# ameli/gaussian-process-param-estimation

Measured on NVIDIA B200. Metric: loglik+grad evals/s (Matern nu=2.5 dense n=20k, FP64), higher is better.
Workload: dtype f64

## Files before the change

gaussian-process-param-estimation_b200/csrc/gp_loglik.cu:

```cuda
#include "../../include/gpgp.h"
#include "gp_common.cuh"
#include "gp_internal.h"
#include "gp_matern.cuh"

namespace gp {

constexpr int MAXP = 16;
constexpr int LMAXD = 8;

__global__ void __launch_bounds__(256)
gram_partial_kernel(const double* __restrict__ A, const double* __restrict__ B, int nrows, int p, int64_t ld,
                    double* partial) {
    __shared__ double sa[64 * MAXP], sb[64 * MAXP];
    const int tid = threadIdx.x;
    const int a = tid / p, b = tid - a * p;
    double acc = 0.0;
    int rows_per_cta = (nrows + gridDim.x - 1) / gridDim.x;
    int r0 = blockIdx.x * rows_per_cta, r1 = min(nrows, r0 + rows_per_cta);
    for (int base = r0; base < r1; base += 64) {
        int cnt = min(64, r1 - base);
        __syncthreads();
        for (int idx = tid; idx < cnt * p; idx += 256) {
            int r = idx / p, c = idx - r * p;
            sa[idx] = A[(int64_t)(base + r) * ld + c];
            sb[idx] = B[(int64_t)(base + r) * ld + c];
        }
        __syncthreads();
        if (tid < p * p)
            for (int r = 0; r < cnt; ++r) acc += sa[r * p + a] * sb[r * p + b];
    }
    if (tid < p * p) partial[(int64_t)blockIdx.x * p * p + tid] = acc;
}

__global__ void sum_partials_kernel(const double* partial, int nparts, int width, double* out) {
    int t = blockIdx.x * blockDim.x + threadIdx.x;
    if (t >= width) return;
    double s = 0.0;
    for (int i = 0; i < nparts; ++i) s += partial[(int64_t)i * width + t];
    out[t] = s;
}

template <int MODE, bool WITH_DK>
__global__ void __launch_bounds__(256)
trace_tiles_kernel(const double* __restrict__ Ainv, int n, int npad, const double* __restrict__ pts, int d,
                   MaternParams mp, double* partial) {
    __shared__ double pr[LMAXD][128], pc[LMAXD][128];
    __shared__ double red[32];
    int b = blockIdx.x;
    int tm = (int)((sqrt(8.0 * b + 1.0) - 1.0) * 0.5);
    while ((tm + 1) * (tm + 2) / 2 <= b) ++tm;
    while (tm * (tm + 1) / 2 > b) --tm;
    int tn = b - tm * (tm + 1) / 2;
    const int m0 = tm * 128, n0 = tn * 128, tid = threadIdx.x;
    if (WITH_DK) {
        for (int idx = tid; idx < 128 * d; idx += 256) {
            int r = idx / d, k = idx - r * d;
            pr[k][r] = (m0 + r < n) ? pts[(int64_t)(m0 + r) * d + k] : 0.0;
            pc[k][r] = (n0 + r < n) ? pts[(int64_t)(n0 + r) * d + k] : 0.0;
        }
        __syncthreads();
    }
    double t1 = 0.0, t2 = 0.0, t3 = 0.0;
    const int tx = tid & 63, ty = tid >> 6;
    for (int r = ty; r < 128; r += 4) {
        int gi = m0 + r;
        if (gi >= n) break;
        double2 v = *reinterpret_cast<const double2*>(Ainv + (int64_t)gi * npad + n0 + 2 * tx);
        double vals[2] = {v.x, v.y};
#pragma unroll
        for (int e = 0; e < 2; ++e) {
            int gj = n0 + 2 * tx + e;
            if (gj > gi || gj >= n) continue;
            double a = vals[e];
            if (gj == gi) {
                t1 += a;
                t2 += a * a;
            } else {
                t2 += 2.0 * a * a;
                if (WITH_DK) {
                    double s = 0.0, ud = 0.0;
#pragma unroll
                    for (int k = 0; k < LMAXD; ++k)
                        if (k < d) {
                            double t = (pr[k][r] - pc[k][2 * tx + e]) * mp.inv_scale[k];
                            s += t * t;
                            if (k == mp.ddim) ud = t * t;
                        }
                    double val, dval;
                    matern_value_drho<MODE>(sqrt(s), mp, &val, &dval);
                    if (mp.ddim >= 0) dval = (s > 0.0) ? dval * (ud / s) * mp.inv_scale[mp.ddim] : 0.0;
                    t3 += 2.0 * a * dval;
                }
            }
        }
    }
    t1 = block_sum(t1, red);
    t2 = block_sum(t2, red);
    t3 = block_sum(t3, red);
    if (tid == 0) {
        partial[(int64_t)b * 3 + 0] = t1;
        partial[(int64_t)b * 3 + 1] = t2;
        partial[(int64_t)b * 3 + 2] = t3;
    }
}

__global__ void __launch_bounds__(256)
frob_lower_kernel(const double* __restrict__ W, int n, int npad, double* partial) {
    __shared__ double red[32];
    int tm = blockIdx.y, tn = blockIdx.x;
    double s = 0.0;
    if (tn <= tm) {
        int m0 = tm * 128, n0 = tn * 128;
        for (int idx = threadIdx.x; idx < 128 * 64; idx += 256) {
            int r = idx >> 6, c = (idx & 63) * 2;
            int gi = m0 + r;
            if (gi >= n) break;
            double2 v = *reinterpret_cast<const double2*>(W + (int64_t)gi * npad + n0 + c);
            if (n0 + c <= gi) s += v.x * v.x;
            if (n0 + c + 1 <= gi) s += v.y * v.y;
        }
    }
    s = block_sum(s, red);
    if (threadIdx.x == 0) partial[blockIdx.y * gridDim.x + blockIdx.x] = s;
}

constexpr int SSP = MAXP + 1;
constexpr int DKR = 16;
template <int MODE, int PP>
__global__ void __launch_bounds__(256)
dk_apply_kernel(const double* __restrict__ pts, int n, int d, MaternParams mp, const double* __restrict__ S, int p,
                int64_t lds, double* __restrict__ V) {
    constexpr int SP = PP + 1;
    __shared__ double pcs[LMAXD][128];
    __shared__ double ss[128 * SP];
    const int tid = threadIdx.x, lane = tid & 31, warp = tid >> 5;
    const int g0 = blockIdx.x * DKR + warp * 2;
    double pi[2][LMAXD];
#pragma unroll
    for (int r = 0; r < 2; ++r)
#pragma unroll
        for (int k = 0; k < LMAXD; ++k) pi[r][k] = (k < d && g0 + r < n) ? pts[(int64_t)(g0 + r) * d + k] : 0.0;
    double acc[2][PP];
#pragma unroll
    for (int r = 0; r < 2; ++r)
#pragma unroll
        for (int c = 0; c < PP; ++c) acc[r][c] = 0.0;
    for (int j0 = 0; j0 < n; j0 += 128) {
        __syncthreads();
        for (int idx = tid; idx < 128 * d; idx += 256) {
            int r = idx / d, k = idx - r * d;
            pcs[k][r] = (j0 + r < n) ? pts[(int64_t)(j0 + r) * d + k] : 0.0;
        }
        for (int idx = tid; idx < 128 * p; idx += 256) {
            int r = idx / p, c = idx - r * p;
            ss[r * SP + c] = (j0 + r < n) ? S[(int64_t)(j0 + r) * lds + c] : 0.0;
        }
        __syncthreads();
#pragma unroll
        for (int t = 0; t < 4; ++t) {
            const int jj = t * 32 + lane;
            const int gj = j0 + jj;
#pragma unroll
            for (int r = 0; r < 2; ++r) {
                const int gi = g0 + r;
                if (gi >= n || gj >= n || gj == gi) continue;
                double s2 = 0.0, ud = 0.0;
#pragma unroll
                for (int k = 0; k < LMAXD; ++k)
                    if (k < d) {
                        double u = (pi[r][k] - pcs[k][jj]) * mp.inv_scale[k];
                        s2 += u * u;
                        if (k == mp.ddim) ud = u * u;
                    }
                double val, dval;
                matern_value_drho<MODE>(sqrt(s2), mp, &val, &dval);
                if (mp.ddim >= 0) dval = (s2 > 0.0) ? dval * (ud / s2) * mp.inv_scale[mp.ddim] : 0.0;
#pragma unroll
                for (int c = 0; c < PP; ++c)
                    if (c < p) acc[r][c] += dval * ss[jj * SP + c];
            }
        }
    }
    const int rows128 = ((n + 127) / 128) * 128;
#pragma unroll
    for (int r = 0; r < 2; ++r)
#pragma unroll
        for (int c = 0; c < PP; ++c)
            if (c < p) {
                const double v = warp_sum(acc[r][c]);
                if (lane == 0 && g0 + r < rows128) V[(int64_t)(g0 + r) * lds + c] = (g0 + r < n) ? v : 0.0;
            }
}

template <int MODE>
static void launch_dk_apply(const double* pts, int n, int d, const MaternParams& mp, const double* S, int p, int64_t lds,
                            double* V, cudaStream_t s) {
    const unsigned grid = (unsigned)((((n + 127) / 128) * 128) / DKR);
    if (p <= 8) dk_apply_kernel<MODE, 8><<<grid, 256, 0, s>>>(pts, n, d, mp, S, p, lds, V);
    else dk_apply_kernel<MODE, MAXP><<<grid, 256, 0, s>>>(pts, n, d, mp, S, p, lds, V);
}

__global__ void __launch_bounds__(256)
symm_skinny_kernel(const double* __restrict__ K, int n, int npad, const double* __restrict__ X, int p, double* __restrict__ Y) {
    __shared__ double xs[128 * SSP];
    const int tid = threadIdx.x, lane = tid & 31, warp = tid >> 5;
    const int r0 = blockIdx.x * 32 + warp * 4;
    double acc[4][MAXP];
#pragma unroll
    for (int r = 0; r < 4; ++r)
#pragma unroll
        for (int c = 0; c < MAXP; ++c) acc[r][c] = 0.0;
    for (int j0 = 0; j0 < npad; j0 += 128) {
        __syncthreads();
        for (int idx = tid; idx < 128 * p; idx += 256) {
            int r = idx / p, c = idx - r * p;
            xs[r * SSP + c] = (j0 + r < n) ? X[(int64_t)(j0 + r) * p + c] : 0.0;
        }
        __syncthreads();
#pragma unroll
        for (int q = 0; q < 4; ++q) {
            int j = lane + 32 * q;
            double kv[4];
#pragma unroll
            for (int r = 0; r < 4; ++r) kv[r] = K[(int64_t)(r0 + r) * npad + j0 + j];
#pragma unroll
            for (int c = 0; c < MAXP; ++c)
                if (c < p) {
                    double x = xs[j * SSP + c];
#pragma unroll
                    for (int r = 0; r < 4; ++r) acc[r][c] += kv[r] * x;
                }
        }
    }
#pragma unroll
    for (int r = 0; r < 4; ++r)
#pragma unroll
        for (int c = 0; c < MAXP; ++c)
            if (c < p) {
                double v = warp_sum(acc[r][c]);
                if (lane == 0) Y[(int64_t)(r0 + r) * p + c] = (r0 + r < n) ? v : 0.0;
            }
}

template <int PP>
__global__ void __launch_bounds__(256)
tril_skinny_kernel(const double* __restrict__ W, int npad, const double* __restrict__ X, int p, double* __restrict__ Y) {
    constexpr int SP = PP + 1;
    __shared__ double xs[128 * SP];
    const int tid = threadIdx.x, lane = tid & 31, warp = tid >> 5;
    const int rb = ((int)gridDim.x - 1 - (int)blockIdx.x) * 32, r0 = rb + warp * 4;
    double acc[4][PP];
#pragma unroll
    for (int r = 0; r < 4; ++r)
#pragma unroll
        for (int c = 0; c < PP; ++c) acc[r][c] = 0.0;
    for (int j0 = 0; j0 < rb + 32; j0 += 128) {
        __syncthreads();
        for (int idx = tid; idx < 128 * p; idx += 256) {
            int r = idx / p, c = idx - r * p;
            xs[r * SP + c] = X[(int64_t)(j0 + r) * p + c];
        }
        __syncthreads();
#pragma unroll
        for (int q = 0; q < 4; ++q) {
            int j = lane + 32 * q;
            double kv[4];
#pragma unroll
            for (int r = 0; r < 4; ++r) kv[r] = (j0 + j <= r0 + r) ? W[(int64_t)(r0 + r) * npad + j0 + j] : 0.0;
#pragma unroll
            for (int c = 0; c < PP; ++c)
                if (c < p) {
                    double x = xs[j * SP + c];
#pragma unroll
                    for (int r = 0; r < 4; ++r) acc[r][c] += kv[r] * x;
                }
        }
    }
#pragma unroll
    for (int r = 0; r < 4; ++r)
#pragma unroll
        for (int c = 0; c < PP; ++c)
            if (c < p) {
                double v = warp_sum(acc[r][c]);
                if (lane == 0) Y[(int64_t)(r0 + r) * p + c] = v;
            }
}

constexpr int TCH = 1024;
template <int PP>
__global__ void __launch_bounds__(256)
trilT_skinny_partial_kernel(const double* __restrict__ W, int npad, const double* __restrict__ X, int p, double* __restrict__ partial) {
    constexpr int SP = PP + 1;
    __shared__ double xs[128 * SP];
    __shared__ double comb[128 * SP];
    const int tid = threadIdx.x;
    const int i0 = blockIdx.x * 128, kc = blockIdx.y;
    const int il = tid & 127, half = tid >> 7, i = i0 + il;
    int kbeg = kc * TCH, kend = min(npad, kbeg + TCH);
    double acc[PP];
#pragma unroll
    for (int c = 0; c < PP; ++c) acc[c] = 0.0;
    if (kend > i0) {
        if (kbeg < i0) kbeg = i0;
        for (int k0 = kbeg; k0 < kend; k0 += 128) {
            __syncthreads();
            for (int idx = tid; idx < 128 * p; idx += 256) {
                int r = idx / p, c = idx - r * p;
                xs[r * SP + c] = X[(int64_t)(k0 + r) * p + c];
            }
            __syncthreads();
#pragma unroll 4
            for (int kk = half; kk < 128; kk += 2) {
                int k = k0 + kk;
                double w = (k >= i) ? W[(int64_t)k * npad + i] : 0.0;
#pragma unroll
                for (int c = 0; c < PP; ++c)
                    if (c < p) acc[c] += w * xs[kk * SP + c];
            }
        }
    }
    __syncthreads();
    if (half == 1)
#pragma unroll
        for (int c = 0; c < PP; ++c) comb[il * SP + c] = acc[c];
    __syncthreads();
    if (half == 0)
        for (int c = 0; c < p; ++c) partial[((int64_t)kc * npad + i) * p + c] = acc[c] + comb[il * SP + c];
}

__global__ void trilT_reduce_kernel(const double* __restrict__ partial, int npad, int p, int nchunks, double* __restrict__ Y) {
    int64_t t = (int64_t)blockIdx.x * blockDim.x + threadIdx.x;
    if (t >= (int64_t)npad * p) return;
    int i = (int)(t / p);
    double s = 0.0;
    for (int kc = i / TCH; kc < nchunks; ++kc) s += partial[(int64_t)kc * npad * p + t];
    Y[t] = s;
}

__global__ void __launch_bounds__(256)
finalize_out_kernel(double* out, const double* logdet, const double* tr_parts, int ntiles, const double* frob_parts,
                    int nfrob, const int* info, int flags) {
    __shared__ double red[32];
    double t1 = 0.0, t2 = 0.0, t3 = 0.0;
    if (flags & 2) {
        for (int i = threadIdx.x; i < ntiles; i += 256) {
            t1 += tr_parts[3 * i];
            t2 += tr_parts[3 * i + 1];
            t3 += tr_parts[3 * i + 2];
        }
    } else if (flags & 1) {
        for (int i = threadIdx.x; i < nfrob; i += 256) t1 += frob_parts[i];
    }
    t1 = block_sum(t1, red);
    t2 = block_sum(t2, red);
    t3 = block_sum(t3, red);
    if (threadIdx.x == 0) {
        out[0] = *logdet;
        out[1] = t1;
        out[2] = t2;
        out[3] = t3;
        out[4] = (double)(*info);
        out[5] = out[6] = out[7] = 0.0;
    }
}

static size_t align256(size_t x) { return (x + 255) & ~(size_t)255; }

struct LoglikWs {
    double* S;
    double* V;
    double* V2;
    double* logdet;
    double* gram;
    double* tr;
    double* frob;
    int* info;
    double* tpart;
    void* potri;
    size_t total;
};

static LoglikWs carve(void* ws, int64_t npad, int p) {
    LoglikWs w;
    char* base = (char*)ws;
    size_t off = 0;
    int64_t T = npad / 128;
    auto take = [&](size_t bytes) { size_t o = off; off += align256(bytes); return base ? base + o : (char*)nullptr; };
    w.S = (double*)take(sizeof(double) * npad * MAXP);
    w.V = (double*)take(sizeof(double) * npad * MAXP);
    w.V2 = (double*)take(sizeof(double) * npad * MAXP);
    w.logdet = (double*)take(sizeof(double) * 4);
    w.gram = (double*)take(sizeof(double) * 296 * MAXP * MAXP);
    w.tr = (double*)take(sizeof(double) * (T * (T + 1) / 2) * 3);
    w.frob = (double*)take(sizeof(double) * T * T);
    w.info = (int*)take(sizeof(int) * 4);
    w.tpart = (double*)take(sizeof(double) * (npad / TCH + 1) * npad * MAXP);
    w.potri = (void*)take((size_t)gp_potri_workspace_bytes(npad));
    w.total = off;
    (void)p;
    return w;
}

static int gram(const double* A, const double* B, int nrows, int p, int64_t ld, double* partial, double* out, cudaStream_t s) {
    int parts = 296;
    gram_partial_kernel<<<parts, 256, 0, s>>>(A, B, nrows, p, ld, partial);
    sum_partials_kernel<<<(p * p + 127) / 128, 128, 0, s>>>(partial, parts, p * p, out);
    GP_COUNT(2);
    GP_LAUNCH_CHECK();
    return 0;
}

static int solve_with_inverse(const double* W, int npad, double* S, double* tmp, int p, double* tpart, cudaStream_t s) {
    int nchunks = (npad + TCH - 1) / TCH;
    if (p <= 8) {
        tril_skinny_kernel<8><<<npad / 32, 256, 0, s>>>(W, npad, S, p, tmp);
        trilT_skinny_partial_kernel<8><<<dim3(npad / 128, nchunks), 256, 0, s>>>(W, npad, tmp, p, tpart);
    } else {
        tril_skinny_kernel<MAXP><<<npad / 32, 256, 0, s>>>(W, npad, S, p, tmp);
        trilT_skinny_partial_kernel<MAXP><<<dim3(npad / 128, nchunks), 256, 0, s>>>(W, npad, tmp, p, tpart);
    }
    trilT_reduce_kernel<<<(unsigned)(((int64_t)npad * p + 255) / 256), 256, 0, s>>>(tpart, npad, p, nchunks, S);
    GP_COUNT(3);
    GP_LAUNCH_CHECK();
    return 0;
}

template <int MODE>
static int grad_reductions(const double* Ainv, int n, int npad, const double* pts, int d, const MaternParams& mp, bool with_dk,
                           const LoglikWs& w, int p, double* outQ, cudaStream_t s) {
    int T = npad / 128, tiles = T * (T + 1) / 2;
    if (with_dk) {
        trace_tiles_kernel<MODE, true><<<tiles, 256, 0, s>>>(Ainv, n, npad, pts, d, mp, w.tr);
        launch_dk_apply<MODE>(pts, n, d, mp, w.S, p, p, w.V, s);
        GP_COUNT(2);
        GP_LAUNCH_CHECK();
        return gram(w.S, w.V, n, p, p, w.gram, outQ, s);
    }
    trace_tiles_kernel<MODE, false><<<tiles, 256, 0, s>>>(Ainv, n, npad, pts, d, mp, w.tr);
    GP_COUNT(1);
    GP_LAUNCH_CHECK();
    return 0;
}

}

using namespace gp;

extern "C" {

int gp_symm_skinny(const double* K, int64_t n, int64_t npad, const double* X, int64_t p, double* Y, void* stream) {
    if (!K || !X || !Y || n <= 0 || npad != gp_padded_size(n) || p <= 0 || p > MAXP) return -1;
    symm_skinny_kernel<<<(unsigned)(npad / 32), 256, 0, (cudaStream_t)stream>>>(K, (int)n, (int)npad, X, (int)p, Y);
    GP_COUNT(1);
    GP_LAUNCH_CHECK();
    return 0;
}

int gp_dk_apply(const double* points, int64_t n, int64_t d, const double* scale_host, double nu, const double* S, int64_t p,
                int64_t lds, double* V, void* stream) {
    if (!points || !scale_host || !S || !V || n <= 0 || d <= 0 || d > LMAXD || p <= 0 || p > MAXP || lds < p) return -1;
    MaternParams mp;
    mp.nu = nu; mp.coef = 0.0; mp.sq2nu = 0.0;
    for (int k = 0; k < d; ++k) {
        if (!(scale_host[k] > 0.0) || scale_host[k] != scale_host[0]) return -4;
        mp.inv_scale[k] = 1.0 / scale_host[k];
    }
    mp.inv_rho = 1.0 / scale_host[0];
    int mode = matern_mode_of(nu);
    if (mode == MAT_GENERAL) {
        mp.coef = pow(2.0, 1.0 - nu) / tgamma(nu);
        mp.sq2nu = sqrt(2.0 * nu);
    }
    cudaStream_t s = (cudaStream_t)stream;
    switch (mode) {
        case MAT_05: launch_dk_apply<MAT_05>(points, (int)n, (int)d, mp, S, (int)p, lds, V, s); break;
        case MAT_15: launch_dk_apply<MAT_15>(points, (int)n, (int)d, mp, S, (int)p, lds, V, s); break;
        case MAT_25: launch_dk_apply<MAT_25>(points, (int)n, (int)d, mp, S, (int)p, lds, V, s); break;
        case MAT_GAUSS: launch_dk_apply<MAT_GAUSS>(points, (int)n, (int)d, mp, S, (int)p, lds, V, s); break;
        default: launch_dk_apply<MAT_GENERAL>(points, (int)n, (int)d, mp, S, (int)p, lds, V, s); break;
    }
    GP_COUNT(1);
    GP_LAUNCH_CHECK();
    return 0;
}

int64_t gp_traces_workspace_bytes(int64_t npad) {
    int64_t T = npad / 128;
    return (int64_t)sizeof(double) * (T * (T + 1) / 2 * 3 + T * T + 64);
}

int gp_inverse_traces(const double* M, int64_t n, int64_t npad, int kind, double* out_dev, void* ws, void* stream) {
    if (!M || !out_dev || !ws || n <= 0 || npad != gp_padded_size(n) || (kind != 0 && kind != 1)) return -1;
    cudaStream_t s = (cudaStream_t)stream;
    int T = (int)(npad / 128), tiles = T * (T + 1) / 2;
    double* tr = (double*)ws;
    double* frob = tr + (int64_t)tiles * 3;
    double* misc = frob + (int64_t)T * T;
    GP_CUDA_CHECK(cudaMemsetAsync(misc, 0, sizeof(double) * 8, s));
    MaternParams mp;
    mp.nu = 0; mp.coef = 0; mp.sq2nu = 0; mp.inv_rho = 0;
    if (kind == 0) frob_lower_kernel<<<dim3(T, T), 256, 0, s>>>(M, (int)n, (int)npad, frob);
    else trace_tiles_kernel<MAT_05, false><<<tiles, 256, 0, s>>>(M, (int)n, (int)npad, nullptr, 0, mp, tr);
    finalize_out_kernel<<<1, 256, 0, s>>>(out_dev, misc, tr, tiles, frob, T * T, (const int*)(misc + 2), kind == 0 ? 1 : 2);
    GP_COUNT(2);
    GP_LAUNCH_CHECK();
    return 0;
}

__global__ void sum_trace3_kernel(const double* __restrict__ tr, int tiles, double* out) {
    __shared__ double red[32];
    double s = 0.0;
    for (int i = threadIdx.x; i < tiles; i += blockDim.x) s += tr[(int64_t)i * 3 + 2];
    s = block_sum(s, red);
    if (threadIdx.x == 0) out[0] = s;
}

int gp_loglik_dense_dscale(const double* Ainv, int64_t n, int64_t npad, int64_t p, const double* points, int64_t d,
                           const double* scale_host, double nu, int64_t dim, void* ws, double* out_dim, void* stream) {
    if (!Ainv || !points || !scale_host || !ws || !out_dim || n <= 0 || npad != gp_padded_size(n) || p <= 0 || p > MAXP ||
        d <= 0 || d > LMAXD || dim < 0 || dim >= d)
        return -1;
    cudaStream_t s = (cudaStream_t)stream;
    LoglikWs w = carve(ws, npad, (int)p);
    MaternParams mp;
    mp.nu = nu; mp.coef = 0.0; mp.sq2nu = 0.0; mp.inv_rho = 1.0; mp.ddim = (int)dim;
    for (int k = 0; k < d; ++k) {
        if (!(scale_host[k] > 0.0)) return -4;
        mp.inv_scale[k] = 1.0 / scale_host[k];
    }
    int mode = matern_mode_of(nu);
    if (mode == MAT_GENERAL) {
        mp.coef = pow(2.0, 1.0 - nu) / tgamma(nu);
        mp.sq2nu = sqrt(2.0 * nu);
    }
    const int N = (int)n, NP = (int)npad, P = (int)p;
    int rc;
    switch (mode) {
        case MAT_05: rc = grad_reductions<MAT_05>(Ainv, N, NP, points, (int)d, mp, true, w, P, out_dim + 1, s); break;
        case MAT_15: rc = grad_reductions<MAT_15>(Ainv, N, NP, points, (int)d, mp, true, w, P, out_dim + 1, s); break;
        case MAT_25: rc = grad_reductions<MAT_25>(Ainv, N, NP, points, (int)d, mp, true, w, P, out_dim + 1, s); break;
        case MAT_GAUSS: rc = grad_reductions<MAT_GAUSS>(Ainv, N, NP, points, (int)d, mp, true, w, P, out_dim + 1, s); break;
        default: rc = grad_reductions<MAT_GENERAL>(Ainv, N, NP, points, (int)d, mp, true, w, P, out_dim + 1, s); break;
    }
    if (rc) return rc;
    int T = NP / 128;
    sum_trace3_kernel<<<1, 256, 0, s>>>(w.tr, T * (T + 1) / 2, out_dim);
    GP_COUNT(1);
    GP_LAUNCH_CHECK();
    return 0;
}

int64_t gp_loglik_workspace_bytes(int64_t npad) { return (int64_t)carve(nullptr, npad, MAXP).total; }

int64_t gp_loglik_out_len(int64_t p) { return 8 + 4 * p * p; }

int gp_loglik_dense(const double* K, int64_t n, int64_t npad, const double* R, int64_t p, double eta, int flags,
                    const double* points, int64_t d, const double* scale_host, double nu, double* A, double* W,
                    void* potrf_ws, void* ws, double* out, void* stream) {
    if (!K || !R || !A || !potrf_ws || !ws || !out || n <= 0 || npad != gp_padded_size(n) || p <= 0 || p > MAXP) return -1;
    if ((flags & 3) && !W) return -2;
    if ((flags & 4) && (!(flags & 2) || !points || !scale_host || d <= 0 || d > LMAXD)) return -3;
    if ((flags & 8) && !(flags & 3)) return -5;
    cudaStream_t s = (cudaStream_t)stream;
    LoglikWs w = carve(ws, npad, (int)p);
    const int N = (int)n, NP = (int)npad, P = (int)p;
    int rc;
    if ((rc = gp_shift_copy(K, n, npad, eta, A, stream))) return rc;
    if ((rc = gp_potrf_f64(A, n, npad, w.info, potrf_ws, stream))) return rc;
    if ((rc = gp_logdet_from_chol(A, n, npad, w.logdet, stream))) return rc;
    GP_CUDA_CHECK(cudaMemcpyAsync(w.S, R, sizeof(double) * npad * p, cudaMemcpyDeviceToDevice, s));
    int T = NP / 128;
    if (flags & 3) {
        if ((rc = gp_trtri_f64(A, W, npad, potrf_ws, w.potri, stream))) return rc;
        if ((rc = solve_with_inverse(W, NP, w.S, w.V, P, w.tpart, s))) return rc;
    } else {
        if ((rc = gp_potrs_f64(A, npad, potrf_ws, w.S, p, p, stream))) return rc;
    }
    double* G = out + 8;
    double* H = G + p * p;
    double* Q = H + p * p;
    if ((rc = gram(R, w.S, N, P, p, w.gram, G, s))) return rc;
    if ((rc = gram(w.S, w.S, N, P, p, w.gram, H, s))) return rc;
    double* T3 = Q + p * p;
    GP_CUDA_CHECK(cudaMemsetAsync(Q, 0, sizeof(double) * 2 * p * p, s));
    if (flags & 8) {
        GP_CUDA_CHECK(cudaMemcpyAsync(w.V2, w.S, sizeof(double) * npad * p, cudaMemcpyDeviceToDevice, s));
        if ((rc = solve_with_inverse(W, NP, w.V2, w.V, P, w.tpart, s))) return rc;
        if ((rc = gram(w.S, w.V2, N, P, p, w.gram, T3, s))) return rc;
    }
    if (flags & 2) {
        if ((rc = gp_lauum_f64(W, A, npad, stream))) return rc;
        bool with_dk = (flags & 4) != 0;
        MaternParams mp;
        mp.nu = nu; mp.coef = 0.0; mp.sq2nu = 0.0; mp.inv_rho = 0.0;
        int mode = MAT_05;
        if (with_dk) {
            for (int k = 0; k < d; ++k) {
                if (!(scale_host[k] > 0.0) || scale_host[k] != scale_host[0]) return -4;
                mp.inv_scale[k] = 1.0 / scale_host[k];
            }
            mp.inv_rho = 1.0 / scale_host[0];
            mode = matern_mode_of(nu);
            if (mode == MAT_GENERAL) {
                mp.coef = pow(2.0, 1.0 - nu) / tgamma(nu);
                mp.sq2nu = sqrt(2.0 * nu);
            }
        }
        switch (mode) {
            case MAT_05: rc = grad_reductions<MAT_05>(A, N, NP, points, (int)d, mp, with_dk, w, P, Q, s); break;
            case MAT_15: rc = grad_reductions<MAT_15>(A, N, NP, points, (int)d, mp, with_dk, w, P, Q, s); break;
            case MAT_25: rc = grad_reductions<MAT_25>(A, N, NP, points, (int)d, mp, with_dk, w, P, Q, s); break;
            case MAT_GAUSS: rc = grad_reductions<MAT_GAUSS>(A, N, NP, points, (int)d, mp, with_dk, w, P, Q, s); break;
            default: rc = grad_reductions<MAT_GENERAL>(A, N, NP, points, (int)d, mp, with_dk, w, P, Q, s); break;
        }
        if (rc) return rc;
    } else if (flags & 1) {
        frob_lower_kernel<<<dim3(T, T), 256, 0, s>>>(W, N, NP, w.frob);
        GP_COUNT(1);
        GP_LAUNCH_CHECK();
    }
    finalize_out_kernel<<<1, 256, 0, s>>>(out, w.logdet, w.tr, T * (T + 1) / 2, w.frob, T * T, w.info, flags);
    GP_COUNT(1);
    GP_LAUNCH_CHECK();
    return 0;
}

}
```

Before: 4.056.

## Fuse derivative-kernel trace with dK·S apply over Ainv lower tiles

```diff
diff --git a/gaussian-process-param-estimation_b200/csrc/gp_loglik.cu b/gaussian-process-param-estimation_b200/csrc/gp_loglik.cu
--- a/gaussian-process-param-estimation_b200/csrc/gp_loglik.cu
+++ b/gaussian-process-param-estimation_b200/csrc/gp_loglik.cu
@@ -2,6 +2,8 @@
 #include "gp_common.cuh"
 #include "gp_internal.h"
 #include "gp_matern.cuh"
+
+#include <algorithm>
 
 namespace gp {
 
@@ -40,11 +42,8 @@
     out[t] = s;
 }
 
-template <int MODE, bool WITH_DK>
 __global__ void __launch_bounds__(256)
-trace_tiles_kernel(const double* __restrict__ Ainv, int n, int npad, const double* __restrict__ pts, int d,
-                   MaternParams mp, double* partial) {
-    __shared__ double pr[LMAXD][128], pc[LMAXD][128];
+trace_tiles_kernel(const double* __restrict__ Ainv, int n, int npad, double* partial) {
     __shared__ double red[32];
     int b = blockIdx.x;
     int tm = (int)((sqrt(8.0 * b + 1.0) - 1.0) * 0.5);
@@ -52,15 +51,7 @@
     while (tm * (tm + 1) / 2 > b) --tm;
     int tn = b - tm * (tm + 1) / 2;
     const int m0 = tm * 128, n0 = tn * 128, tid = threadIdx.x;
-    if (WITH_DK) {
-        for (int idx = tid; idx < 128 * d; idx += 256) {
-            int r = idx / d, k = idx - r * d;
-            pr[k][r] = (m0 + r < n) ? pts[(int64_t)(m0 + r) * d + k] : 0.0;
-            pc[k][r] = (n0 + r < n) ? pts[(int64_t)(n0 + r) * d + k] : 0.0;
-        }
-        __syncthreads();
-    }
-    double t1 = 0.0, t2 = 0.0, t3 = 0.0;
+    double t1 = 0.0, t2 = 0.0;
     const int tx = tid & 63, ty = tid >> 6;
     for (int r = ty; r < 128; r += 4) {
         int gi = m0 + r;
@@ -77,30 +68,15 @@
                 t2 += a * a;
             } else {
                 t2 += 2.0 * a * a;
-                if (WITH_DK) {
-                    double s = 0.0, ud = 0.0;
-#pragma unroll
-                    for (int k = 0; k < LMAXD; ++k)
-                        if (k < d) {
-                            double t = (pr[k][r] - pc[k][2 * tx + e]) * mp.inv_scale[k];
-                            s += t * t;
-                            if (k == mp.ddim) ud = t * t;
-                        }
-                    double val, dval;
-                    matern_value_drho<MODE>(sqrt(s), mp, &val, &dval);
-                    if (mp.ddim >= 0) dval = (s > 0.0) ? dval * (ud / s) * mp.inv_scale[mp.ddim] : 0.0;
-                    t3 += 2.0 * a * dval;
-                }
             }
         }
     }
     t1 = block_sum(t1, red);
     t2 = block_sum(t2, red);
-    t3 = block_sum(t3, red);
     if (tid == 0) {
         partial[(int64_t)b * 3 + 0] = t1;
         partial[(int64_t)b * 3 + 1] = t2;
-        partial[(int64_t)b * 3 + 2] = t3;
+        partial[(int64_t)b * 3 + 2] = 0.0;
     }
 }
 
@@ -200,6 +176,161 @@
     else dk_apply_kernel<MODE, MAXP><<<grid, 256, 0, s>>>(pts, n, d, mp, S, p, lds, V);
 }
 
+__device__ __forceinline__ double transpose_sum16(double (&v)[16], int lane) {
+#pragma unroll
+    for (int h = 8; h >= 1; h >>= 1) {
+        const int o = 2 * h;
+        const bool up = (lane & o) != 0;
+#pragma unroll
+        for (int i = 0; i < h; ++i) {
+            const double send = up ? v[i] : v[i + h];
+            const double keep = up ? v[i + h] : v[i];
+            v[i] = keep + __shfl_xor_sync(0xffffffffu, send, o);
+        }
+    }
+    return v[0] + __shfl_xor_sync(0xffffffffu, v[0], 1);
+}
+
+template <int MODE, int PP>
+__global__ void __launch_bounds__(256, PP <= 8 ? 2 : 1)
+dk_trace_apply_kernel(const double* __restrict__ Ainv, int n, int npad, const double* __restrict__ pts, int d,
+                      MaternParams mp, const double* __restrict__ S, int p, double* __restrict__ tr,
+                      double* __restrict__ vpart) {
+    constexpr int CW = 16 / PP;
+    extern __shared__ __align__(16) double dsm[];
+    double* pr = dsm;
+    double* pc = pr + d * 128;
+    double* ssr = pc + d * 128;
+    double* ssc = ssr + PP * 128;
+    double* rstage = ssc + PP * 128;
+    const int T = npad / 128;
+    const int b = blockIdx.x;
+    int tm = (int)((sqrt(8.0 * b + 1.0) - 1.0) * 0.5);
+    while ((tm + 1) * (tm + 2) / 2 <= b) ++tm;
+    while (tm * (tm + 1) / 2 > b) --tm;
+    const int tn = b - tm * (tm + 1) / 2;
+    const int m0 = tm * 128, n0 = tn * 128, tid = threadIdx.x, lane = tid & 31, warp = tid >> 5;
+    for (int idx = tid; idx < 128 * d; idx += 256) {
+        int r = idx / d, k = idx - r * d;
+        pr[k * 128 + r] = (m0 + r < n) ? pts[(int64_t)(m0 + r) * d + k] : 0.0;
+        pc[k * 128 + r] = (n0 + r < n) ? pts[(int64_t)(n0 + r) * d + k] : 0.0;
+    }
+    for (int idx = tid; idx < 128 * PP; idx += 256) {
+        int r = idx / PP, c = idx - r * PP;
+        ssr[c * 128 + r] = (c < p && m0 + r < n) ? S[(int64_t)(m0 + r) * p + c] : 0.0;
+        ssc[r * PP + c] = (c < p && n0 + r < n) ? S[(int64_t)(n0 + r) * p + c] : 0.0;
+    }
+    __syncthreads();
+
+    double t1 = 0.0, t2 = 0.0, t3 = 0.0;
+    double csum[16 / CW];
+#pragma unroll
+    for (int ch = 0; ch < 16 / CW; ++ch) csum[ch] = 0.0;
+    double* rowblk = vpart + ((int64_t)tm * (T + 1) + tn) * 128 * p;
+#pragma unroll 1
+    for (int q = 0; q < 4; ++q) {
+        const int r = lane + 32 * q, gi = m0 + r;
+        double sr[PP], racc[PP];
+#pragma unroll
+        for (int c = 0; c < PP; ++c) {
+            sr[c] = ssr[c * 128 + r];
+            racc[c] = 0.0;
+        }
+#pragma unroll
+        for (int ch = 0; ch < 16 / CW; ++ch) {
+            const int jc0 = warp * 16 + ch * CW;
+            double v[16];
+#pragma unroll
+            for (int i = 0; i < 16; ++i) v[i] = 0.0;
+            double a[CW];
+#pragma unroll
+            for (int jj = 0; jj < CW; ++jj) a[jj] = (gi < n) ? __ldg(Ainv + (int64_t)gi * npad + n0 + jc0 + jj) : 0.0;
+#pragma unroll
+            for (int jj = 0; jj < CW; ++jj) {
+                const int jc = jc0 + jj, gj = n0 + jc;
+                if (gi >= n || gj >= n || gj > gi) continue;
+                const double av = a[jj];
+                if (gj == gi) {
+                    t1 += av;
+                    t2 += av * av;
+                    continue;
+                }
+                t2 += 2.0 * av * av;
+                double s = 0.0, ud = 0.0;
+#pragma unroll
+                for (int k = 0; k < LMAXD; ++k)
+                    if (k < d) {
+                        double u = (pr[k * 128 + r] - pc[k * 128 + jc]) * mp.inv_scale[k];
+                        s += u * u;
+                        if (k == mp.ddim) ud = u * u;
+                    }
+                double val, dval;
+                matern_value_drho<MODE>(sqrt(s), mp, &val, &dval);
+                if (mp.ddim >= 0) dval = (s > 0.0) ? dval * (ud / s) * mp.inv_scale[mp.ddim] : 0.0;
+                t3 += 2.0 * av * dval;
+#pragma unroll
+                for (int c = 0; c < PP; ++c) {
+                    racc[c] += dval * ssc[jc * PP + c];
+                    v[jj * PP + c] += dval * sr[c];
+                }
+            }
+            csum[ch] += transpose_sum16(v, lane);
+        }
+#pragma unroll
+        for (int c = 0; c < PP; ++c) rstage[(warp * PP + c) * 32 + lane] = racc[c];
+        __syncthreads();
+        for (int idx = tid; idx < 32 * p; idx += 256) {
+            const int rl = idx / p, c = idx - rl * p;
+            double sum = 0.0;
+            for (int w = 0; w < 8; ++w) sum += rstage[(w * PP + c) * 32 + rl];
+            rowblk[(int64_t)(32 * q + rl) * p + c] = sum;
+        }
+        __syncthreads();
+    }
+    double* colblk = vpart + ((int64_t)tn * (T + 1) + (tn == tm ? T : tm)) * 128 * p;
+#pragma unroll
+    for (int ch = 0; ch < 16 / CW; ++ch) {
+        const int m = lane >> 1, jj = m / PP, c = m % PP;
+        if (!(lane & 1) && c < p) colblk[(int64_t)(warp * 16 + ch * CW + jj) * p + c] = csum[ch];
+    }
+    t1 = block_sum(t1, pr);
+    t2 = block_sum(t2, pr);
+    t3 = block_sum(t3, pr);
+    if (tid == 0) {
+        tr[(int64_t)b * 3 + 0] = t1;
+        tr[(int64_t)b * 3 + 1] = t2;
+        tr[(int64_t)b * 3 + 2] = t3;
+    }
+}
+
+__global__ void vpart_reduce_kernel(const double* __restrict__ vpart, int n, int npad, int p, double* __restrict__ V) {
+    const int64_t t = (int64_t)blockIdx.x * blockDim.x + threadIdx.x;
+    if (t >= (int64_t)npad * p) return;
+    const int i = (int)(t / p), c = (int)(t - (int64_t)i * p), I = i / 128, T = npad / 128;
+    double s = 0.0;
+    if (i < n) {
+        const double* src = vpart + (int64_t)I * (T + 1) * 128 * p + (i % 128) * p + c;
+        for (int J = 0; J <= T; ++J) s += src[(int64_t)J * 128 * p];
+    }
+    V[t] = s;
+}
+
+template <int MODE>
+static void launch_dk_trace_apply(const double* Ainv, int n, int npad, const double* pts, int d, const MaternParams& mp,
+                                  const double* S, int p, double* tr, double* vpart, double* V, cudaStream_t s) {
+    const int T = npad / 128, tiles = T * (T + 1) / 2;
+    if (p <= 8) {
+        const int smem = (int)sizeof(double) * 128 * (2 * d + 4 * 8);
+        configure_once((const void*)dk_trace_apply_kernel<MODE, 8>, (int)sizeof(double) * 128 * (2 * LMAXD + 4 * 8));
+        dk_trace_apply_kernel<MODE, 8><<<tiles, 256, smem, s>>>(Ainv, n, npad, pts, d, mp, S, p, tr, vpart);
+    } else {
+        const int smem = (int)sizeof(double) * 128 * (2 * d + 4 * MAXP);
+        configure_once((const void*)dk_trace_apply_kernel<MODE, MAXP>, (int)sizeof(double) * 128 * (2 * LMAXD + 4 * MAXP));
+        dk_trace_apply_kernel<MODE, MAXP><<<tiles, 256, smem, s>>>(Ainv, n, npad, pts, d, mp, S, p, tr, vpart);
+    }
+    vpart_reduce_kernel<<<(unsigned)(((int64_t)npad * p + 255) / 256), 256, 0, s>>>(vpart, n, npad, p, V);
+}
+
 __global__ void __launch_bounds__(256)
 symm_skinny_kernel(const double* __restrict__ K, int n, int npad, const double* __restrict__ X, int p, double* __restrict__ Y) {
     __shared__ double xs[128 * SSP];
@@ -242,38 +373,50 @@
             }
 }
 
+constexpr int TRC = 256;
+constexpr int QB = 4;
 template <int PP>
-__global__ void __launch_bounds__(256)
+__global__ void __launch_bounds__(256, PP <= 8 ? 2 : 1)
 tril_skinny_kernel(const double* __restrict__ W, int npad, const double* __restrict__ X, int p, double* __restrict__ Y) {
     constexpr int SP = PP + 1;
-    __shared__ double xs[128 * SP];
+    __shared__ double xs[TRC * SP];
     const int tid = threadIdx.x, lane = tid & 31, warp = tid >> 5;
     const int rb = ((int)gridDim.x - 1 - (int)blockIdx.x) * 32, r0 = rb + warp * 4;
+    const int jlim = ((rb + 32 + 127) / 128) * 128;
     double acc[4][PP];
 #pragma unroll
     for (int r = 0; r < 4; ++r)
 #pragma unroll
         for (int c = 0; c < PP; ++c) acc[r][c] = 0.0;
-    for (int j0 = 0; j0 < rb + 32; j0 += 128) {
-        __syncthreads();
-        for (int idx = tid; idx < 128 * p; idx += 256) {
+    for (int j0 = 0; j0 < jlim; j0 += TRC) {
+        __syncthreads();
+        for (int idx = tid; idx < TRC * p; idx += 256) {
             int r = idx / p, c = idx - r * p;
-            xs[r * SP + c] = X[(int64_t)(j0 + r) * p + c];
-        }
-        __syncthreads();
-#pragma unroll
-        for (int q = 0; q < 4; ++q) {
-            int j = lane + 32 * q;
-            double kv[4];
-#pragma unroll
-            for (int r = 0; r < 4; ++r) kv[r] = (j0 + j <= r0 + r) ? W[(int64_t)(r0 + r) * npad + j0 + j] : 0.0;
-#pragma unroll
-            for (int c = 0; c < PP; ++c)
-                if (c < p) {
-                    double x = xs[j * SP + c];
-#pragma unroll
-                    for (int r = 0; r < 4; ++r) acc[r][c] += kv[r] * x;
+            xs[r * SP + c] = (j0 + r < npad) ? X[(int64_t)(j0 + r) * p + c] : 0.0;
+        }
+        __syncthreads();
+#pragma unroll
+        for (int qb = 0; qb < TRC / 32; qb += QB) {
+            if (j0 + 32 * qb >= jlim) break;
+            double kv[QB][4];
+#pragma unroll
+            for (int q = 0; q < QB; ++q)
+#pragma unroll
+                for (int r = 0; r < 4; ++r) {
+                    const int j = j0 + lane + 32 * (qb + q);
+                    kv[q][r] = (j <= r0 + r) ? __ldg(W + (int64_t)(r0 + r) * npad + j) : 0.0;
                 }
+#pragma unroll
+            for (int q = 0; q < QB; ++q) {
+                const int j = lane + 32 * (qb + q);
+#pragma unroll
+                for (int c = 0; c < PP; ++c)
+                    if (c < p) {
+                        double x = xs[j * SP + c];
+#pragma unroll
+                        for (int r = 0; r < 4; ++r) acc[r][c] += kv[q][r] * x;
+                    }
+            }
         }
     }
 #pragma unroll
@@ -377,6 +520,7 @@
     int* info;
     double* tpart;
     void* potri;
+    double* vpart;
     size_t total;
 };
 
@@ -395,7 +539,8 @@
     w.frob = (double*)take(sizeof(double) * T * T);
     w.info = (int*)take(sizeof(int) * 4);
     w.tpart = (double*)take(sizeof(double) * (npad / TCH + 1) * npad * MAXP);
-    w.potri = (void*)take((size_t)gp_potri_workspace_bytes(npad));
+    w.potri = (void*)take(std::max((size_t)gp_potri_workspace_bytes(npad), sizeof(double) * T * (T + 1) * 128 * MAXP));
+    w.vpart = (double*)w.potri;
     w.total = off;
     (void)p;
     return w;
@@ -430,13 +575,12 @@
                            const LoglikWs& w, int p, double* outQ, cudaStream_t s) {
     int T = npad / 128, tiles = T * (T + 1) / 2;
     if (with_dk) {
-        trace_tiles_kernel<MODE, true><<<tiles, 256, 0, s>>>(Ainv, n, npad, pts, d, mp, w.tr);
-        launch_dk_apply<MODE>(pts, n, d, mp, w.S, p, p, w.V, s);
+        launch_dk_trace_apply<MODE>(Ainv, n, npad, pts, d, mp, w.S, p, w.tr, w.vpart, w.V, s);
         GP_COUNT(2);
         GP_LAUNCH_CHECK();
         return gram(w.S, w.V, n, p, p, w.gram, outQ, s);
     }
-    trace_tiles_kernel<MODE, false><<<tiles, 256, 0, s>>>(Ainv, n, npad, pts, d, mp, w.tr);
+    trace_tiles_kernel<<<tiles, 256, 0, s>>>(Ainv, n, npad, w.tr);
     GP_COUNT(1);
     GP_LAUNCH_CHECK();
     return 0;
@@ -497,10 +641,8 @@
     double* frob = tr + (int64_t)tiles * 3;
     double* misc = frob + (int64_t)T * T;
     GP_CUDA_CHECK(cudaMemsetAsync(misc, 0, sizeof(double) * 8, s));
-    MaternParams mp;
-    mp.nu = 0; mp.coef = 0; mp.sq2nu = 0; mp.inv_rho = 0;
     if (kind == 0) frob_lower_kernel<<<dim3(T, T), 256, 0, s>>>(M, (int)n, (int)npad, frob);
-    else trace_tiles_kernel<MAT_05, false><<<tiles, 256, 0, s>>>(M, (int)n, (int)npad, nullptr, 0, mp, tr);
+    else trace_tiles_kernel<<<tiles, 256, 0, s>>>(M, (int)n, (int)npad, tr);
     finalize_out_kernel<<<1, 256, 0, s>>>(out_dev, misc, tr, tiles, frob, T * T, (const int*)(misc + 2), kind == 0 ? 1 : 2);
     GP_COUNT(2);
     GP_LAUNCH_CHECK();
```

Result: no change. 4.092 (median of 6 runs) (+0.9%).
